# NVlabs/FB-BEV

Measured on NVIDIA B200. Metric: bev_voxels_per_sec, higher is better.
Workload: dtype f32

## Files before the change

### fb-bev_b200/_lib.py

```python
import ctypes
import os
import subprocess

import torch

_HERE = os.path.dirname(os.path.abspath(__file__))
LIB_PATH = os.environ.get("FBBEV_LIB") or os.path.join(
    _HERE, "lib", "libfbbev_b200.so")
CSRC_DIR = os.path.join(_HERE, "csrc")

_p = ctypes.c_void_p
_i32 = ctypes.c_int32
_i64 = ctypes.c_int64
_sz = ctypes.c_size_t

_SIGNATURES = {
    "fbbev_abi_version": (ctypes.c_int, []),
    "fbbev_debug_launch_count": (ctypes.c_longlong, []),
    "fbbev_error_string": (ctypes.c_char_p, [ctypes.c_int]),
    "fbbev_bev_pool_v2_fwd": (ctypes.c_int, [_p] * 7 + [_i32, _i32, _p, _p]),
    "fbbev_bev_pool_v2_dense_workspace_bytes": (
        _sz, [_i32, _i64, _i32, _i32, _i32]),
    "fbbev_bev_pool_v2_fwd_dense": (
        ctypes.c_int,
# ... 49 lines not shown
                              [_p] + [_i32] * 9 + [_p, _p, _sz, _p]),
    "fbbev_history_warp": (ctypes.c_int, [_p, _i64, _p] + [_i32] * 5 +
                           [_p, _i32, _i32, _p]),
    "fbbev_linear_packed_bytes": (ctypes.c_size_t, [_i32, _i32]),
    "fbbev_linear_pack": (ctypes.c_int, [_p, _i32, _i32, _p, _p]),
    "fbbev_linear_fwd_split": (ctypes.c_int, [
        _p, _i64, _p, _i64, _p, _p, _i64, _i32, _i32, _i32, _i32, _p, _i64, _p,
        _i64, _p]),
    "fbbev_linear_fwd": (ctypes.c_int, [
        _p, _i64, _p, _p, _p, _i64, _p, _p, _i64, _i32, _i32, _i32,
        ctypes.c_float, _p, _i64, _p]),
    "fbbev_ffn_supported": (ctypes.c_int, [_i32, _i32]),
    "fbbev_ffn_fwd": (ctypes.c_int, [
        _p, _i64, _p, _p, _p, _p, _p, _i64, _p, _p, _i64, _i32, _i32,
        ctypes.c_float, _p, _i64, _p]),
}
EXPORTED_SYMBOLS = tuple(_SIGNATURES)

ABI_VERSION = 4
_lib = None


class FbbevError(RuntimeError):
    pass


def build(verbose=False):
    cmd = ["make", "-C", CSRC_DIR, "-j", str(min(8, os.cpu_count() or 1))]
    res = subprocess.run(cmd, stdout=subprocess.PIPE, stderr=subprocess.STDOUT,
                         text=True)
# ... 112 lines not shown
```

### fb-bev_b200/csrc/ffn_tf32.cu

```cuda
#include "common.cuh"
#include "tc5.cuh"

namespace fbbev {
namespace ffn {

constexpr int kKB = 40;
constexpr int kChunks = kKB / 4;
constexpr int kTileM = 128;
constexpr int kAPart = kTileM * kKB * 4;
constexpr int kABlock = 2 * kAPart;
constexpr int kAChunkStride = (kTileM / 8) * 128;
constexpr int kThreads = 448;
constexpr int kHC = 80;
constexpr int kMaxE = 80;
constexpr int kMaxHidden = 320;
constexpr int kTmemCols = 512;
constexpr int kSmemLimit = 232448 - 1024;
constexpr int kCtrlBytes = 512 + (kMaxHidden + 3 * kMaxE) * 4;
constexpr int kSlabBytes = kTileM * (kMaxE + 4) * 4;

#ifdef FFN_TRACE
constexpr int kTraceCap = 200;
__device__ long long g_ffn_trace[5 * 2 * kTraceCap];
__device__ int g_ffn_trace_cnt[5];
#define FTRACE_DECL int trn_ = 0;
#define FTRACE_L(lane_, tag)                                                 \
  do {                                                                       \
    if (blockIdx.x == 0 && trn_ < kTraceCap) {                               \
      g_ffn_trace[(lane_) * 2 * kTraceCap + 2 * trn_] = (tag);               \
      g_ffn_trace[(lane_) * 2 * kTraceCap + 2 * trn_ + 1] = clock64();       \
      g_ffn_trace_cnt[lane_] = ++trn_;                                       \
    }                                                                        \
  } while (0)
#else
#define FTRACE_DECL
#define FTRACE_L(lane_, tag) do {} while (0)
#endif

struct Params {
  const float* x;
  const float* w1p;
  const float* b1;
  const float* w2p;
  const float* b2;
  const float* residual;
  const float* gamma;
  const float* beta;
  float* y;
  int M, E, hidden, npad, n_kb1, n_kb2, n_hc, rows_per_cta, wstages;
  int64_t ldx, ldr, ldy;
  float eps;
};

__global__ void __launch_bounds__(kThreads, 1) ffn_tf32_kernel(const Params p) {
  extern __shared__ __align__(1024) unsigned char smem[];
  FTRACE_DECL
  const int warp = threadIdx.x >> 5, lane = threadIdx.x & 31;
  const int npad = p.npad, S = p.wstages;
  const uint32_t w1_stage = 2u * kHC * kKB * 4;
  const uint32_t w2_stage = 2u * (uint32_t)npad * kKB * 4;
  const uint32_t wstage = w1_stage > w2_stage ? w1_stage : w2_stage;
  unsigned char* xa = smem;
  unsigned char* slab_raw = smem + 2 * kABlock;
  unsigned char* wr = slab_raw + kSlabBytes;
  unsigned char* ctrl = wr + (size_t)S * wstage;
  const uint32_t bars = smem_u32(ctrl);
  const uint32_t bar_xfull = bars, bar_xempty = bars + 8;
  const uint32_t bar_yfull = bars + 16, bar_yempty = bars + 24;
  const uint32_t bar_hafull = bars + 32;
  const uint32_t bar_haempty = bars + 48;
  const uint32_t bar_hfull = bars + 64;
  const uint32_t bar_wfull = bars + 128;
  const uint32_t bar_wempty = bars + 160;
  uint32_t* tmem_slot = reinterpret_cast<uint32_t*>(ctrl + 192);
  float* s_b1 = reinterpret_cast<float*>(ctrl + 512);
  float* s_b2 = s_b1 + kMaxHidden;
  float* s_gamma = s_b2 + kMaxE;
  float* s_beta = s_gamma + kMaxE;
  const uint32_t xa_base = smem_u32(xa), wr_base = smem_u32(wr);

  if (warp == 12) {
    if (lane == 0) {
      mbar_init(bar_xfull, 128);
      mbar_init(bar_xempty, 1);
      mbar_init(bar_yfull, 1);
      mbar_init(bar_yempty, 128);
      for (int g = 0; g < 2; ++g) {
        mbar_init(bar_hafull + 8u * g, 128);
        mbar_init(bar_haempty + 8u * g, 1);
      }
      for (int c = 0; c < p.n_hc; ++c) mbar_init(bar_hfull + 8u * c, 1);
      for (int s = 0; s < S; ++s) {
        mbar_init(bar_wfull + 8u * s, 1);
        mbar_init(bar_wempty + 8u * s, 1);
      }
      fence_mbar_init();
    }
    __syncwarp();
    asm volatile(
        "tcgen05.alloc.cta_group::1.sync.aligned.shared::cta.b32 [%0], %1;" ::"r"(
            smem_u32(tmem_slot)),
        "r"(kTmemCols)
        : "memory");
    asm volatile("tcgen05.relinquish_alloc_permit.cta_group::1.sync.aligned;" ::
                     : "memory");
  }
  for (int j = threadIdx.x; j < kMaxHidden; j += kThreads)
    s_b1[j] = (p.b1 && j < p.hidden) ? p.b1[j] : 0.f;
  for (int j = threadIdx.x; j < kMaxE; j += kThreads) {
    s_b2[j] = (p.b2 && j < p.E) ? p.b2[j] : 0.f;
    s_gamma[j] = (p.gamma && j < p.E) ? p.gamma[j] : 1.f;
    s_beta[j] = (p.beta && j < p.E) ? p.beta[j] : 0.f;
  }
  tc_fence_before();
  __syncthreads();
  tc_fence_after();
  const uint32_t tmem_base = *tmem_slot;
  if (threadIdx.x == 0) FTRACE_L(4, 1);
  const int row_begin = blockIdx.x * p.rows_per_cta;
  const int row_end = min(p.M, row_begin + p.rows_per_cta);
  const int n_my = row_end > row_begin ? (row_end - row_begin + kTileM - 1) / kTileM : 0;
  const int stages_per_tile = p.n_hc * p.n_kb1 + p.n_kb2;

  if (warp >= 4 && warp < 8) {
    const int lw = warp - 4;
    const int r_lo = lane & 15, c_lo = lane >> 4;
    auto load_x = [&](int ti) {
      float4 v[2][10];
#pragma unroll
      for (int u = 0; u < 2; ++u) {
        const int g0 = row_begin + ti * kTileM + lw * 32 + r_lo;
        const int col0 = u * kKB + 4 * c_lo;
        const float* b0 = p.x + (size_t)g0 * p.ldx + col0;
        const float* b1 = b0 + (size_t)16 * p.ldx;
        const bool ok0 = u < p.n_kb1 && g0 < row_end;
        const bool ok1 = u < p.n_kb1 && g0 + 16 < row_end;
#pragma unroll
// ... 25 lines not shown
          lo.x = x.x - hi.x; lo.y = x.y - hi.y;
          lo.z = x.z - hi.z; lo.w = x.w - hi.w;
          const uint32_t off =
              (uint32_t)(ch * (kTileM / 8) + (row >> 3)) * 128u + (row & 7) * 16u;
          unsigned char* a = xa + (size_t)u * kABlock + off;
          *reinterpret_cast<float4*>(a) = hi;
          *reinterpret_cast<float4*>(a + kAPart) = lo;
        }
      }
      fence_proxy_async();
      mbar_arrive(bar_xfull);
      if (threadIdx.x == 128) FTRACE_L(0, 120 + ti);
    };
    for (int ti = 0; ti < n_my; ++ti) load_x(ti);
  } else if (warp == 13) {
    const int n_w1 = p.n_hc * p.n_kb1;
    uint32_t it = 0;
    for (int ti = 0; ti < n_my; ++ti) {
      for (int j = 0; j < stages_per_tile; ++j, ++it) {
        const uint32_t s = it % S, ph = (it / S) & 1u;
        const float* src;
        uint32_t bytes;
        if (j < n_w1) {
          src = p.w1p + (size_t)j * (w1_stage / 4u);
          bytes = w1_stage;
        } else {
          src = p.w2p + (size_t)(j - n_w1) * (w2_stage / 4u);
          bytes = w2_stage;
        }
        mbar_wait(bar_wempty + 8u * s, ph ^ 1u);
        if (lane == 0) FTRACE_L(1, 1000 + it);
        if (elect_one()) {
          mbar_arrive_expect_tx(bar_wfull + 8u * s, bytes);
          bulk_g2s(wr_base + s * wstage, src, bytes, bar_wfull + 8u * s);
        }
        __syncwarp();
      }
    }
  } else if (warp == 12) {
    {
      const uint32_t idesc1 = (1u << 4) | (2u << 7) | (2u << 10) |
                              ((uint32_t)(kHC >> 3) << 17) | (8u << 24);
      const uint32_t idesc2 = (1u << 4) | (2u << 7) | (2u << 10) |
                              ((uint32_t)(npad >> 3) << 17) | (8u << 24);
      const uint32_t lbo_b1 = (uint32_t)kHC * 16u, lbo_b2 = (uint32_t)npad * 16u;
      const uint32_t w1_part = (uint32_t)kHC * kKB * 4;
      const uint32_t w2_part = (uint32_t)npad * kKB * 4;
      const uint32_t d_y = tmem_base + (uint32_t)p.hidden;
      const uint32_t d_lo = d_y + (uint32_t)npad;
      uint32_t it = 0, hu = 0;
      for (int ti = 0; ti < n_my; ++ti) {
        if (lane == 0) FTRACE_L(2, 200 + ti);
        mbar_wait(bar_xfull, ti & 1);
        tc_fence_after();
        if (lane == 0) FTRACE_L(2, 210 + ti);
        for (int c = 0; c < p.n_hc; ++c) {
          const uint32_t d = tmem_base + (uint32_t)(c * kHC);
          for (int kb = 0; kb < p.n_kb1; ++kb, ++it) {
            const uint32_t s = it % S, ph = (it / S) & 1u;
            mbar_wait(bar_wfull + 8u * s, ph);
            tc_fence_after();
            if (lane == 0) FTRACE_L(2, 2000 + it);
            const uint32_t a_hi = xa_base + (uint32_t)kb * kABlock;
            const uint32_t a_lo = a_hi + kAPart;
            const uint32_t w_hi = wr_base + s * wstage;
            const uint32_t w_lo = w_hi + w1_part;
            if (elect_one()) {
#pragma unroll
// ... 7 lines not shown
              mma_tf32(d, dal, dbh, idesc1, 1u);
              mma_tf32(d, dah, dbl, idesc1, 1u);
            }
            tc_commit(bar_wempty + 8u * s);
            if (kb == p.n_kb1 - 1) {
              tc_commit(bar_hfull + 8u * c);
              if (c == p.n_hc - 1) tc_commit(bar_xempty);
            }
            }
            __syncwarp();
          }
        }
        mbar_wait(bar_yempty, (ti & 1) ^ 1);
        tc_fence_after();
        for (int kb = 0; kb < p.n_kb2; ++kb, ++it, ++hu) {
          const uint32_t s = it % S, ph = (it / S) & 1u;
          const uint32_t g = (uint32_t)kb & 1u, hph = (hu >> 1) & 1u;
          mbar_wait(bar_wfull + 8u * s, ph);
          if (lane == 0) FTRACE_L(2, 2000 + it);
          mbar_wait(bar_hafull + 8u * g, hph);
          tc_fence_after();
          if (lane == 0) FTRACE_L(2, 3000 + it);
          const uint32_t a_hi = tmem_base + (uint32_t)(kb * kKB);
          const uint32_t a_lo = d_lo + g * (uint32_t)kKB;
          const uint32_t w_hi = wr_base + s * wstage;
          const uint32_t w_lo = w_hi + w2_part;
          if (elect_one()) {
#pragma unroll
          for (int k = 0; k < kChunks / 2; ++k) {
            const uint32_t bo = 2u * k * lbo_b2;
            const uint64_t dbh = smem_desc(w_hi + bo, lbo_b2, 128);
            const uint64_t dbl = smem_desc(w_lo + bo, lbo_b2, 128);
            mma_tf32_ts(d_y, a_hi + 8u * k, dbh, idesc2, (kb | k) != 0);
            mma_tf32_ts(d_y, a_lo + 8u * k, dbh, idesc2, 1u);
            mma_tf32_ts(d_y, a_hi + 8u * k, dbl, idesc2, 1u);
          }
          tc_commit(bar_wempty + 8u * s);
          tc_commit(bar_haempty + 8u * g);
          if (kb == p.n_kb2 - 1) tc_commit(bar_yfull);
          }
          __syncwarp();
        }
        if (lane == 0) FTRACE_L(2, 220 + ti);
      }
    }
    __syncwarp();
  } else if (warp != 13) {
    const uint32_t grp = warp >> 3;
    const int q = warp & 3;
    const int gt = q * 32 + lane;
    const uint32_t lane_base = tmem_base + ((uint32_t)(q * 32) << 16);
    const int E = p.E;
    if (grp == 1) {
      const uint32_t t_lo = lane_base + (uint32_t)(p.hidden + npad);
      uint32_t use = 0;
      for (int ti = 0; ti < n_my; ++ti) {
        for (int kb = 0; kb < p.n_kb2; ++kb, ++use) {
// ... 24 lines not shown
          tmem_st16(tl, lo);
          tmem_st16(tl + 16u, lo + 16);
          tmem_st8(tl + 32u, lo + 32);
          tmem_st_wait();
          tc_fence_before();
          mbar_arrive(bar_hafull + 8u * g);
          if (threadIdx.x == 256) FTRACE_L(3, 6000 + use);
        }
      }
    } else {
      const int pitch = E + 4;
      float* slab = reinterpret_cast<float*>(slab_raw);
      float* my_row = slab + (size_t)gt * pitch;
      const uint32_t ty = lane_base + (uint32_t)p.hidden;
      const int nc16 = npad >> 4;
      for (int ti = 0; ti < n_my; ++ti) {
        const int row0 = row_begin + ti * kTileM;
        const bool in_range = row0 + gt < row_end;
        bulk_wait_read0();
        asm volatile("bar.sync 1, 128;" ::: "memory");
        if (p.residual) {
          const int crow = gt >> 2, cq = gt & 3;
#pragma unroll 1
          for (int c = 0; c < nc16; ++c) {
            const int col = 16 * c + 4 * cq;
#pragma unroll
            for (int i = 0; i < 4; ++i) {
              const int r = crow + 32 * i;
              const bool ok = row0 + r < row_end && col < E;
              const float* src = p.residual +
                                 (size_t)(ok ? row0 + r : row_begin) * p.ldr +
                                 (ok ? col : 0);
              const uint32_t dst = smem_u32(slab + (size_t)r * pitch + col);
              asm volatile("cp.async.cg.shared.global [%0], [%1], 16, %2;" ::"r"(dst),
                           "l"(src), "r"(ok ? 16 : 0)
                           : "memory");
            }
          }
          asm volatile("cp.async.commit_group;" ::: "memory");
        }
        if (threadIdx.x == 0) FTRACE_L(4, 300 + ti);
        mbar_wait(bar_yfull, ti & 1);
        tc_fence_after();
        if (threadIdx.x == 0) FTRACE_L(4, 310 + ti);
        if (p.residual) {
          asm volatile("cp.async.wait_group 0;" ::: "memory");
          asm volatile("bar.sync 1, 128;" ::: "memory");
        }
        float sum = 0.f, sq = 0.f, shiftK = 0.f;
#pragma unroll 1
        for (int c = 0; c < nc16; ++c) {
          float v[16];
          tmem_ld16(ty + 16u * c, v);
          tmem_ld_wait();
          if (c == nc16 - 1) {
            tc_fence_before();
            mbar_arrive(bar_yempty);
          }
#pragma unroll
          for (int j = 0; j < 4; ++j) {
            const int col = 16 * c + 4 * j;
            if (col < E) {
              const float4 bb = *reinterpret_cast<const float4*>(s_b2 + col);
              float4 t = make_float4(v[4 * j] + bb.x, v[4 * j + 1] + bb.y,
                                     v[4 * j + 2] + bb.z, v[4 * j + 3] + bb.w);
              float4* cell = reinterpret_cast<float4*>(my_row + col);
              if (p.residual) {
                const float4 r = *cell;
                t.x += r.x; t.y += r.y; t.z += r.z; t.w += r.w;
              }
              *cell = t;
              if (col == 0) shiftK = t.x;
              const float a = t.x - shiftK, b = t.y - shiftK, cc = t.z - shiftK,
                          d = t.w - shiftK;
              sum += (a + b) + (cc + d);
              sq += (a * a + b * b) + (cc * cc + d * d);
            }
          }
        }
        if (p.gamma) {
          const float dm = sum / (float)E;
          const float mean = shiftK + dm;
          const float var = fmaxf(sq / (float)E - dm * dm, 0.f);
          const float rstd = rsqrtf(var + p.eps);
          const float4* g4 = reinterpret_cast<const float4*>(s_gamma);
          const float4* b4 = reinterpret_cast<const float4*>(s_beta);
#pragma unroll 4
          for (int j = 0; j < (E >> 2); ++j) {
            float4* cell = reinterpret_cast<float4*>(my_row + 4 * j);
            const float4 t = *cell, g = g4[j], b = b4[j];
            *cell = make_float4(fmaf((t.x - mean) * rstd, g.x, b.x),
                                fmaf((t.y - mean) * rstd, g.y, b.y),
                                fmaf((t.z - mean) * rstd, g.z, b.z),
                                fmaf((t.w - mean) * rstd, g.w, b.w));
          }
        }
        if (in_range) {
          fence_proxy_async();
          bulk_s2g(p.y + (size_t)(row0 + gt) * p.ldy, smem_u32(my_row),
                   (uint32_t)E * 4u);
        }
        bulk_commit();
        if (threadIdx.x == 0) FTRACE_L(4, 320 + ti);
      }
      bulk_wait0();
      if (threadIdx.x == 0) FTRACE_L(4, 330);
    }
  }

  tc_fence_before();
  __syncthreads();
// ... 19 lines not shown
  cudaMemcpyFromSymbol(out, ffn::g_ffn_trace,
                       sizeof(long long) * 5 * 2 * ffn::kTraceCap);
  return ffn::kTraceCap;
}
#endif

FBBEV_API int fbbev_ffn_supported(int32_t embed, int32_t hidden) {
  return embed > 0 && embed <= ffn::kMaxE && embed % 4 == 0 && hidden > 0 &&
                 hidden % ffn::kHC == 0 &&
                 hidden + ffn::pad16(embed) + 2 * ffn::kKB <= ffn::kTmemCols &&
                 hidden <= ffn::kMaxHidden
             ? 1
             : 0;
}

FBBEV_API int fbbev_ffn_fwd(const float* x, int64_t ldx, const float* w1_packed,
                            const float* b1, const float* w2_packed,
                            const float* b2, const float* residual, int64_t ldr,
                            const float* ln_weight, const float* ln_bias,
                            int64_t m, int32_t embed, int32_t hidden,
                            float ln_eps, float* y, int64_t ldy,
                            fbbev_stream_t stream) {
  if (!x || !w1_packed || !w2_packed || !y || m < 0)
    return FBBEV_ERR_INVALID_ARGUMENT;
  if ((ln_weight == nullptr) != (ln_bias == nullptr))
    return FBBEV_ERR_INVALID_ARGUMENT;
  if (!fbbev_ffn_supported(embed, hidden) || m > (int64_t)1 << 30)
    return FBBEV_ERR_UNSUPPORTED;
  if (ldx < embed || ldy < embed || (residual && ldr < embed) || ldx % 4 ||
      ldy % 4 || (residual && ldr % 4))
    return FBBEV_ERR_INVALID_ARGUMENT;
  if ((reinterpret_cast<uintptr_t>(x) | reinterpret_cast<uintptr_t>(y) |
       reinterpret_cast<uintptr_t>(w1_packed) |
       reinterpret_cast<uintptr_t>(w2_packed) |
       reinterpret_cast<uintptr_t>(residual)) & 15)
    return FBBEV_ERR_INVALID_ARGUMENT;
  if (m == 0) return FBBEV_OK;
  ffn::Params p;
  p.x = x; p.w1p = w1_packed; p.b1 = b1; p.w2p = w2_packed; p.b2 = b2;
  p.residual = residual; p.gamma = ln_weight; p.beta = ln_bias; p.y = y;
  p.M = (int)m; p.E = embed; p.hidden = hidden; p.npad = ffn::pad16(embed);
  p.n_kb1 = (embed + ffn::kKB - 1) / ffn::kKB;
  p.n_kb2 = hidden / ffn::kKB;
  p.n_hc = hidden / ffn::kHC;
  p.ldx = ldx; p.ldr = ldr; p.ldy = ldy; p.eps = ln_eps;
  const size_t w1_stage = 2 * (size_t)ffn::kHC * ffn::kKB * 4;
  const size_t w2_stage = 2 * (size_t)p.npad * ffn::kKB * 4;
  const size_t wstage = w1_stage > w2_stage ? w1_stage : w2_stage;
  const size_t fixed =
      2 * (size_t)ffn::kABlock + ffn::kSlabBytes + ffn::kCtrlBytes;
  int S = (int)((ffn::kSmemLimit - fixed) / wstage);
  S = S > 4 ? 4 : S;
  if (S < 2) return FBBEV_ERR_UNSUPPORTED;
  p.wstages = S;
  const size_t smem = fixed + (size_t)S * wstage;
  static int n_sm = 0;
  if (n_sm == 0) {
    int dev = 0;
    cudaGetDevice(&dev);
    cudaDeviceGetAttribute(&n_sm, cudaDevAttrMultiProcessorCount, dev);
    if (n_sm <= 0) n_sm = 148;
  }
  const int n_tiles = (int)ceil_div64(m, ffn::kTileM);
  const int tiles_per_cta = (int)ceil_div64(n_tiles, n_sm);
  p.rows_per_cta = tiles_per_cta * ffn::kTileM;
  const int grid = (int)ceil_div64(m, p.rows_per_cta);
  static size_t allowed = 0;
  if (smem > allowed) {
    cudaError_t e = cudaFuncSetAttribute(
        ffn::ffn_tf32_kernel, cudaFuncAttributeMaxDynamicSharedMemorySize,
        (int)smem);
    if (e != cudaSuccess) return (int)e;
    allowed = smem;
  }
  count_launch();
  ffn::ffn_tf32_kernel<<<grid, ffn::kThreads, smem, as_stream(stream)>>>(p);
  return launch_status();
}
```

### fb-bev_b200/csrc/linear_tf32.cu

```cuda
#include "common.cuh"
#include "tc5.cuh"

namespace fbbev {

constexpr int kKB = 40;
constexpr int kChunks = kKB / 4;
constexpr int kTileM = 128;
constexpr int kAPart = kTileM * kKB * 4;
constexpr int kAChunkStride = (kTileM / 8) * 128;
constexpr int kLinThreads = 448;
constexpr int kMaxN = 192;
constexpr int kTmemCols = 512;
constexpr int kSmemLimit = 232448 - 1024;
constexpr int kSlabPitch = 20;
constexpr int kSlabBytes = 2 * kTileM * kSlabPitch * 4;
constexpr int kCtrlBytes = 256 + 3 * kMaxN * 4;

#ifdef LIN_TRACE
__device__ long long g_trace[512];
__device__ int g_trace_n;
#define TRACE_DECL __shared__ long long s_trace[8][64]; __shared__ int s_trace_n[8];
#define TRACE(lane_, tag)                                                    \
  do {                                                                       \
    if (blockIdx.x == 0) {                                                   \
// ... 256 lines not shown
    for (int ti = 0; ti < n_my; ++ti, ++tc) {
      if ((tc & 1u) != grp) continue;
      const uint32_t aph = (tc >> 1) & 1u;
      const int row0 = row_begin + ti * kTileM;
      const uint32_t taddr =
          tmem_base + ((uint32_t)(q * 32) << 16) + grp * (uint32_t)npad;
      if (LN) {
        bulk_wait_read0();
        group_sync();
        if (p.residual) {
#pragma unroll 1
          for (int c = 0; c < nc16; ++c) {
            const int col = 16 * c + 4 * cq;
#pragma unroll
            for (int i = 0; i < 4; ++i) {
              const int r = crow + 32 * i;
              const bool ok = row0 + r < row_end && col < N;
              const float* src = p.residual +
                                 (size_t)(ok ? row0 + r : row_begin) * p.ldr +
                                 (ok ? col : 0);
              const uint32_t dst = smem_u32(slab + (size_t)r * pitch + col);
              asm volatile("cp.async.cg.shared.global [%0], [%1], 16, %2;" ::"r"(dst),
                           "l"(src), "r"(ok ? 16 : 0)
                           : "memory");
            }
          }
          asm volatile("cp.async.commit_group;" ::: "memory");
        }
        if (gt == 0) TRACE(3 + grp, 600 + tc);
        mbar_wait(bar_tfull + 8u * grp, aph);
        tc_fence_after();
        if (gt == 0) TRACE(3 + grp, 700 + tc);
// ... 286 lines not shown
```

### fb-bev_b200/ops/linear.py

```python
import torch

from .. import _lib

MAX_N = 192


def _pack(weight):
    key = (weight.data_ptr(), weight._version, tuple(weight.shape), weight.device)
    hit = getattr(weight, "_fbbev_packed", None)
    if hit is not None and hit[0] == key:
        return hit[1]
    L = _lib.lib()
    n, k = weight.shape
    w = weight.detach().contiguous().float()
    blocks = []
    for n0 in range(0, n, MAX_N):
        n1 = min(n, n0 + MAX_N)
        nbytes = L.fbbev_linear_packed_bytes(n1 - n0, k)
        buf = torch.empty(nbytes // 4, dtype=torch.float32, device=w.device)
        _lib.check(L.fbbev_linear_pack(_lib.ptr(w[n0:n1]), n1 - n0, k, _lib.ptr(buf),
                                       _lib.stream_ptr(w.device)), "fbbev_linear_pack")
        blocks.append((n0, n1, buf))
    try:
        weight._fbbev_packed = (key, blocks)
# ... 149 lines not shown
    w1p = _pack_ffn_w1(w1)
    (_, _, w2p), = _pack(w2)
    _lib.check(_lib.lib().fbbev_ffn_fwd(
        _lib.ptr(x2), x2.stride(0), _lib.ptr(w1p),
        _lib.ptr(b1.detach().contiguous()) if b1 is not None else None,
        _lib.ptr(w2p),
        _lib.ptr(b2.detach().contiguous()) if b2 is not None else None,
        _lib.ptr(r2), r2.stride(0) if r2 is not None else 0,
        _lib.ptr(ln_weight) if ln_weight is not None else None,
        _lib.ptr(ln_bias) if ln_bias is not None else None,
        m, embed, hidden, float(eps), _lib.ptr(y), y.stride(0),
        _lib.stream_ptr(x.device)), "fbbev_ffn_fwd")
    return y.view(*lead, embed)


class LinearTF32Function(torch.autograd.Function):

    @staticmethod
    def forward(ctx, x, weight, bias, relu, residual):
        assert not (relu and residual is not None)
        y = linear_fused(
            x.detach(), weight.detach(),
            None if bias is None else bias.detach(), relu=relu,
            residual=None if residual is None else residual.detach())
        ctx.relu = relu
        ctx.has_bias = bias is not None
        ctx.has_res = residual is not None
        ctx.save_for_backward(x, weight, y if relu else None)
        return y

# ... 23 lines not shown
```

### fb-bev_b200/view_transformation/backward_projection.py

```python
import copy
import math
import os
import warnings

import torch
import torch.nn as nn
import torch.nn.functional as F

from ..ops import linear as _linear_ops
from .forward_projection import inv3x3_many
from ..ops import ms_deform_attn as _msda_ops
from ..ops.ms_deform_attn import (MultiScaleDeformableAttnFunction_fp32,
                                  bev_mask_fold,
                                  da_spatial_cross_attention_core,
                                  da_spatial_cross_attention_core_autograd,
                                  ms_deform_attn_fused, ms_deform_attn_unfused,
                                  needs_grad)
from ..registry import (BaseModule, build_attention,
                        build_feedforward_network, build_positional_encoding,
                        build_transformer, build_transformer_layer,
                        build_transformer_layer_sequence, register)

__all__ = ['BackwardProjection', 'BEVFormer', 'bevformer_encoder',
           'BEVFormerEncoderLayer', 'MyCustomBaseTransformerLayer',
# ... 427 lines not shown
        if self.layer_scale is None and _fused_linear_on(slots, self.dropout):
            return _linear(self.output_proj, slots, residual=inp_residual,
                           norm=post_norm)
        slots = self.output_proj(slots)
        if self.layer_scale is None:
            out = self.dropout(slots) + inp_residual
        else:
            out = self.dropout(self.layer_scale * slots) + inp_residual
        return out if post_norm is None else post_norm(out)

    def forward(self, query, key, value, residual=None, query_pos=None,
                key_padding_mask=None, reference_points=None,
                spatial_shapes=None, reference_points_cam=None,
                level_start_index=None, flag='encoder', bev_query_depth=None,
                pred_img_depth=None, bev_mask=None, per_cam_mask_list=None,
                post_norm=None, **kwargs):
        query = query.float()
        if key is None:
            key = query
        if value is None:
            value = key
        inp_residual = query if residual is None else residual
        side_event = kwargs.get('side_event')
        if side_event is not None and query.is_cuda:
            torch.cuda.current_stream(query.device).wait_event(side_event)
        sca_prepared = (kwargs.get('sca_prepared') or {}).get(id(self))
        if bev_mask is not None:
            if self.rebatch_bev_mask or not query.is_cuda:
                if query_pos is not None:
                    query = query + query_pos.float()
                return self._forward_rebatch(
                    query, value, inp_residual, key_padding_mask,
                    spatial_shapes, reference_points_cam, level_start_index,
                    bev_query_depth, pred_img_depth, bev_mask,
                    per_cam_mask_list, post_norm)
            per_cam_mask_list = bev_mask_fold(per_cam_mask_list, bev_mask)
            sca_prepared = None

        da = self.deformable_attention
        B, N, DC, H, W = pred_img_depth.shape
        depth_prob = pred_img_depth.reshape(B * N, DC, H * W).permute(0, 2, 1)
        v = (kwargs.get('projected_values') or {}).get(id(self))
        if v is None:
# ... 1 lines not shown
        offsets, logits = da.project_query(
            query, None if query_pos is None else query_pos.float())
        if bev_query_depth.dim() == 5:
            bev_query_depth = bev_query_depth[..., 0]
        if needs_grad(v, depth_prob, offsets, logits):
            slots = da_spatial_cross_attention_core_autograd(
                v, depth_prob, reference_points_cam, bev_query_depth,
                per_cam_mask_list, offsets, logits, spatial_shapes,
                level_start_index, self.dbound, da.num_Z_anchors)
        else:
            slots = da_spatial_cross_attention_core(
                v, depth_prob, reference_points_cam, bev_query_depth,
                per_cam_mask_list, offsets, logits, spatial_shapes,
                level_start_index, self.dbound, da.num_Z_anchors,
                prepared=sca_prepared)
        return self._finish(slots, inp_residual, post_norm)

    def project_camera_value(self, value):
        num_cams, n_value, bs, E = value.shape
        value = value.permute(2, 0, 1, 3).reshape(bs * num_cams, n_value, E)
        return self.deformable_attention.project_value(value.float())

    def _forward_rebatch(self, query, value, inp_residual, key_padding_mask,
                         spatial_shapes, reference_points_cam,
                         level_start_index, bev_query_depth, pred_img_depth,
                         bev_mask, per_cam_mask_list, post_norm=None):
        N, B, nq, Z, _ = bev_query_depth.shape
        _, _, DC, H, W = pred_img_depth.shape
        depth_q = bev_query_depth.permute(1, 0, 2, 3, 4)
        depth_prob = pred_img_depth.reshape(B * N, DC, H * W).permute(0, 2, 1)
# ... 160 lines not shown
                    attn_mask=attn_masks[attn_index],
                    key_padding_mask=bev_mask, reference_points=ref_2d,
                    spatial_shapes=_const_tensor(((bev_h, bev_w),),
                                                 query.device),
                    level_start_index=_const_tensor((0,), query.device),
                    post_norm=fold, bev_w=bev_w, **kwargs)
                attn_index += 1
                identity = query
                skip_norm = fold is not None
            elif op == 'norm':
                if not skip_norm:
                    query = self.norms[norm_index](query)
                skip_norm = False
                norm_index += 1
            elif op == 'cross_attn':
                query = self.attentions[attn_index](
                    query, key, value, identity if self.pre_norm else None,
                    query_pos=bev_pos, key_pos=key_pos,
                    reference_points=ref_3d,
                    reference_points_cam=reference_points_cam,
                    attn_mask=attn_masks[attn_index],
                    key_padding_mask=key_padding_mask,
                    spatial_shapes=spatial_shapes,
                    level_start_index=level_start_index,
                    bev_query_depth=bev_query_depth,
                    pred_img_depth=pred_img_depth, bev_mask=bev_mask,
                    per_cam_mask_list=per_cam_mask_list, post_norm=fold,
                    **kwargs)
                attn_index += 1
                identity = query
                skip_norm = fold is not None
            elif op == 'ffn':
                query = self.ffns[ffn_index](
                    query, identity if self.pre_norm else None,
                    post_norm=fold)
                ffn_index += 1
                skip_norm = fold is not None
        return query


@register('TRANSFORMER_LAYER_SEQUENCE')
class bevformer_encoder(BaseModule):

    fused_geometry = os.environ.get('FBBEV_EXACT_GEOMETRY', '0') != '1'
    side_stream = os.environ.get('FBBEV_SIDE_STREAM', '1') == '1'

    @staticmethod
    def _side(device):
        key = str(device)
        if key not in _SIDE_STREAMS:
            _SIDE_STREAMS[key] = torch.cuda.Stream(device=device)
        return _SIDE_STREAMS[key]

# ... 302 lines not shown
```

### include/fbbev_b200.h

```cpp
#ifndef FBBEV_B200_H_
#define FBBEV_B200_H_

#include <stddef.h>
#include <stdint.h>

#ifdef __cplusplus
extern "C" {
#endif

#define FBBEV_OK 0
#define FBBEV_ERR_INVALID_ARGUMENT (-1)
#define FBBEV_ERR_WORKSPACE_TOO_SMALL (-2)
#define FBBEV_ERR_UNSUPPORTED (-3)

#define FBBEV_ABI_VERSION 4

typedef void* fbbev_stream_t;

int fbbev_abi_version(void);
long long fbbev_debug_launch_count(void);
const char* fbbev_error_string(int code);


int fbbev_bev_pool_v2_fwd(const float* depth, const float* feat,
// ... 189 lines not shown
int fbbev_linear_fwd_split(const float* x, int64_t ldx, const float* x_add,
                           int64_t ldx_add, const float* packed,
                           const float* bias, int64_t m, int32_t k, int32_t n,
                           int32_t n_split, int32_t relu, float* y0,
                           int64_t ldy0, float* y1, int64_t ldy1,
                           fbbev_stream_t stream);

int fbbev_ffn_supported(int32_t embed, int32_t hidden);
int fbbev_ffn_fwd(const float* x, int64_t ldx, const float* w1_packed,
                  const float* b1, const float* w2_packed, const float* b2,
                  const float* residual, int64_t ldr, const float* ln_weight,
                  const float* ln_bias, int64_t m, int32_t embed,
                  int32_t hidden, float ln_eps, float* y, int64_t ldy,
                  fbbev_stream_t stream);


int fbbev_history_warp(const float* history, int64_t history_batch_stride,
                       const float* flow, int32_t n, int32_t mc, int32_t Z,
                       int32_t H, int32_t W, float* out, int32_t c_total,
                       int32_t ch_offset, fbbev_stream_t stream);

#ifdef __cplusplus
}
#endif
#endif
```

Before: 1.549 billion.

## Fuse cross-attention output projection and LayerNorm into the FFN tcgen05 kernel

Adds a prologue GEMM stage to the TF32 FFN kernel that computes the cross-attention output projection, adds the bias and residual, and applies the first LayerNorm. The normalized rows are written back as the FFN input and residual, and the next tile's prologue is interleaved with the current tile's second GEMM. The encoder layer routes cross_attn, norm, ffn and norm through this single kernel when the configuration matches. This removes a separate linear launch and the global round trip of the intermediate activation. In exchange it adds extra pipeline barriers, shared-memory control space, and ordering complexity between the bulk stores and the residual reloads.

```diff
diff --git a/fb-bev_b200/_lib.py b/fb-bev_b200/_lib.py
--- a/fb-bev_b200/_lib.py
+++ b/fb-bev_b200/_lib.py
@@ -87,6 +87,9 @@
     "fbbev_ffn_fwd": (ctypes.c_int, [
         _p, _i64, _p, _p, _p, _p, _p, _i64, _p, _p, _i64, _i32, _i32,
         ctypes.c_float, _p, _i64, _p]),
+    "fbbev_proj_ln_ffn_fwd": (ctypes.c_int, [
+        _p, _i64, _p, _p, _p, _i64, _p, _p, ctypes.c_float, _p, _p, _p, _p,
+        _p, _p, _i64, _i32, _i32, ctypes.c_float, _p, _i64, _p]),
 }
 EXPORTED_SYMBOLS = tuple(_SIGNATURES)
 
diff --git a/fb-bev_b200/csrc/ffn_tf32.cu b/fb-bev_b200/csrc/ffn_tf32.cu
--- a/fb-bev_b200/csrc/ffn_tf32.cu
+++ b/fb-bev_b200/csrc/ffn_tf32.cu
@@ -16,7 +16,7 @@
 constexpr int kMaxHidden = 320;
 constexpr int kTmemCols = 512;
 constexpr int kSmemLimit = 232448 - 1024;
-constexpr int kCtrlBytes = 512 + (kMaxHidden + 3 * kMaxE) * 4;
+constexpr int kCtrlBytes = 512 + (kMaxHidden + 6 * kMaxE) * 4;
 constexpr int kSlabBytes = kTileM * (kMaxE + 4) * 4;
 
 #ifdef FFN_TRACE
@@ -47,9 +47,14 @@
   const float* gamma;
   const float* beta;
   float* y;
+  const float* wop;
+  const float* bo;
+  const float* residual0;
+  const float* gamma0;
+  const float* beta0;
   int M, E, hidden, npad, n_kb1, n_kb2, n_hc, rows_per_cta, wstages;
-  int64_t ldx, ldr, ldy;
-  float eps;
+  int64_t ldx, ldr, ldy, ldr0;
+  float eps, eps0;
 };
 
 __global__ void __launch_bounds__(kThreads, 1) ffn_tf32_kernel(const Params p) {
@@ -70,6 +75,8 @@
   const uint32_t bar_hafull = bars + 32;
   const uint32_t bar_haempty = bars + 48;
   const uint32_t bar_hfull = bars + 64;
+  const uint32_t bar_pfull = bars + 112;
+  const uint32_t bar_qfull = bars + 120;
   const uint32_t bar_wfull = bars + 128;
   const uint32_t bar_wempty = bars + 160;
   uint32_t* tmem_slot = reinterpret_cast<uint32_t*>(ctrl + 192);
@@ -77,6 +84,10 @@
   float* s_b2 = s_b1 + kMaxHidden;
   float* s_gamma = s_b2 + kMaxE;
   float* s_beta = s_gamma + kMaxE;
+  float* s_bo = s_beta + kMaxE;
+  float* s_gamma0 = s_bo + kMaxE;
+  float* s_beta0 = s_gamma0 + kMaxE;
+  const bool pro = p.wop != nullptr;
   const uint32_t xa_base = smem_u32(xa), wr_base = smem_u32(wr);
 
   if (warp == 12) {
@@ -90,6 +101,8 @@
         mbar_init(bar_haempty + 8u * g, 1);
       }
       for (int c = 0; c < p.n_hc; ++c) mbar_init(bar_hfull + 8u * c, 1);
+      mbar_init(bar_pfull, 1);
+      mbar_init(bar_qfull, 128);
       for (int s = 0; s < S; ++s) {
         mbar_init(bar_wfull + 8u * s, 1);
         mbar_init(bar_wempty + 8u * s, 1);
@@ -111,6 +124,9 @@
     s_b2[j] = (p.b2 && j < p.E) ? p.b2[j] : 0.f;
     s_gamma[j] = (p.gamma && j < p.E) ? p.gamma[j] : 1.f;
     s_beta[j] = (p.beta && j < p.E) ? p.beta[j] : 0.f;
+    s_bo[j] = (p.bo && j < p.E) ? p.bo[j] : 0.f;
+    s_gamma0[j] = (p.gamma0 && j < p.E) ? p.gamma0[j] : 1.f;
+    s_beta0[j] = (p.beta0 && j < p.E) ? p.beta0[j] : 0.f;
   }
   tc_fence_before();
   __syncthreads();
@@ -120,7 +136,8 @@
   const int row_begin = blockIdx.x * p.rows_per_cta;
   const int row_end = min(p.M, row_begin + p.rows_per_cta);
   const int n_my = row_end > row_begin ? (row_end - row_begin + kTileM - 1) / kTileM : 0;
-  const int stages_per_tile = p.n_hc * p.n_kb1 + p.n_kb2;
+  const int n_w0 = pro ? p.n_kb1 : 0;
+  const int stages_per_tile = n_w0 + p.n_hc * p.n_kb1 + p.n_kb2;
 
   if (warp >= 4 && warp < 8) {
     const int lw = warp - 4;
@@ -176,27 +193,30 @@
     };
     for (int ti = 0; ti < n_my; ++ti) load_x(ti);
   } else if (warp == 13) {
-    const int n_w1 = p.n_hc * p.n_kb1;
     uint32_t it = 0;
+    auto issue = [&](const float* src, uint32_t bytes) {
+      const uint32_t s = it % S, ph = (it / S) & 1u;
+      mbar_wait(bar_wempty + 8u * s, ph ^ 1u);
+      if (lane == 0) FTRACE_L(1, 1000 + it);
+      if (elect_one()) {
+        mbar_arrive_expect_tx(bar_wfull + 8u * s, bytes);
+        bulk_g2s(wr_base + s * wstage, src, bytes, bar_wfull + 8u * s);
+      }
+      __syncwarp();
+      ++it;
+    };
+    auto issue_wo = [&]() {
+      for (int kb = 0; kb < p.n_kb1; ++kb)
+        issue(p.wop + (size_t)kb * (w2_stage / 4u), w2_stage);
+    };
+    if (pro && n_my > 0) issue_wo();
     for (int ti = 0; ti < n_my; ++ti) {
-      for (int j = 0; j < stages_per_tile; ++j, ++it) {
-        const uint32_t s = it % S, ph = (it / S) & 1u;
-        const float* src;
-        uint32_t bytes;
-        if (j < n_w1) {
-          src = p.w1p + (size_t)j * (w1_stage / 4u);
-          bytes = w1_stage;
-        } else {
-          src = p.w2p + (size_t)(j - n_w1) * (w2_stage / 4u);
-          bytes = w2_stage;
-        }
-        mbar_wait(bar_wempty + 8u * s, ph ^ 1u);
-        if (lane == 0) FTRACE_L(1, 1000 + it);
-        if (elect_one()) {
-          mbar_arrive_expect_tx(bar_wfull + 8u * s, bytes);
-          bulk_g2s(wr_base + s * wstage, src, bytes, bar_wfull + 8u * s);
-        }
-        __syncwarp();
+      for (int j = 0; j < p.n_hc * p.n_kb1; ++j)
+        issue(p.w1p + (size_t)j * (w1_stage / 4u), w1_stage);
+      for (int kb = 0; kb <= p.n_kb2; ++kb) {
+        if (kb == 2 && pro && ti + 1 < n_my) issue_wo();
+        if (kb == p.n_kb2) break;
+        issue(p.w2p + (size_t)kb * (w2_stage / 4u), w2_stage);
       }
     }
   } else if (warp == 12) {
@@ -211,9 +231,39 @@
       const uint32_t d_y = tmem_base + (uint32_t)p.hidden;
       const uint32_t d_lo = d_y + (uint32_t)npad;
       uint32_t it = 0, hu = 0;
+      auto gemm0 = [&](int t) {
+        mbar_wait(bar_xfull, t & 1);
+        tc_fence_after();
+        for (int kb = 0; kb < p.n_kb1; ++kb, ++it) {
+          const uint32_t s = it % S, ph = (it / S) & 1u;
+          mbar_wait(bar_wfull + 8u * s, ph);
+          tc_fence_after();
+          const uint32_t a_hi = xa_base + (uint32_t)kb * kABlock;
+          const uint32_t a_lo = a_hi + kAPart;
+          const uint32_t w_hi = wr_base + s * wstage;
+          const uint32_t w_lo = w_hi + w2_part;
+          if (elect_one()) {
+#pragma unroll
+          for (int k = 0; k < kChunks / 2; ++k) {
+            const uint32_t ao = 2u * k * kAChunkStride, bo = 2u * k * lbo_b2;
+            const uint64_t dah = smem_desc(a_hi + ao, kAChunkStride, 128);
+            const uint64_t dal = smem_desc(a_lo + ao, kAChunkStride, 128);
+            const uint64_t dbh = smem_desc(w_hi + bo, lbo_b2, 128);
+            const uint64_t dbl = smem_desc(w_lo + bo, lbo_b2, 128);
+            mma_tf32(tmem_base, dah, dbh, idesc2, (kb | k) != 0);
+            mma_tf32(tmem_base, dal, dbh, idesc2, 1u);
+            mma_tf32(tmem_base, dah, dbl, idesc2, 1u);
+          }
+          tc_commit(bar_wempty + 8u * s);
+          if (kb == p.n_kb1 - 1) tc_commit(bar_pfull);
+          }
+          __syncwarp();
+        }
+      };
+      if (pro && n_my > 0) gemm0(0);
       for (int ti = 0; ti < n_my; ++ti) {
         if (lane == 0) FTRACE_L(2, 200 + ti);
-        mbar_wait(bar_xfull, ti & 1);
+        mbar_wait(pro ? bar_qfull : bar_xfull, ti & 1);
         tc_fence_after();
         if (lane == 0) FTRACE_L(2, 210 + ti);
         for (int c = 0; c < p.n_hc; ++c) {
@@ -251,6 +301,7 @@
         mbar_wait(bar_yempty, (ti & 1) ^ 1);
         tc_fence_after();
         for (int kb = 0; kb < p.n_kb2; ++kb, ++it, ++hu) {
+          if (kb == 2 && pro && ti + 1 < n_my) gemm0(ti + 1);
           const uint32_t s = it % S, ph = (it / S) & 1u;
           const uint32_t g = (uint32_t)kb & 1u, hph = (hu >> 1) & 1u;
           mbar_wait(bar_wfull + 8u * s, ph);
@@ -278,6 +329,7 @@
           }
           __syncwarp();
         }
+        if (p.n_kb2 == 2 && pro && ti + 1 < n_my) gemm0(ti + 1);
         if (lane == 0) FTRACE_L(2, 220 + ti);
       }
     }
@@ -332,58 +384,49 @@
       float* my_row = slab + (size_t)gt * pitch;
       const uint32_t ty = lane_base + (uint32_t)p.hidden;
       const int nc16 = npad >> 4;
-      for (int ti = 0; ti < n_my; ++ti) {
-        const int row0 = row_begin + ti * kTileM;
-        const bool in_range = row0 + gt < row_end;
-        bulk_wait_read0();
-        asm volatile("bar.sync 1, 128;" ::: "memory");
-        if (p.residual) {
-          const int crow = gt >> 2, cq = gt & 3;
+      auto prefetch_rows = [&](const float* src0, int64_t ld, int row0) {
+        const int crow = gt >> 2, cq = gt & 3;
 #pragma unroll 1
-          for (int c = 0; c < nc16; ++c) {
-            const int col = 16 * c + 4 * cq;
-#pragma unroll
-            for (int i = 0; i < 4; ++i) {
-              const int r = crow + 32 * i;
-              const bool ok = row0 + r < row_end && col < E;
-              const float* src = p.residual +
-                                 (size_t)(ok ? row0 + r : row_begin) * p.ldr +
-                                 (ok ? col : 0);
-              const uint32_t dst = smem_u32(slab + (size_t)r * pitch + col);
-              asm volatile("cp.async.cg.shared.global [%0], [%1], 16, %2;" ::"r"(dst),
-                           "l"(src), "r"(ok ? 16 : 0)
-                           : "memory");
-            }
-          }
-          asm volatile("cp.async.commit_group;" ::: "memory");
-        }
-        if (threadIdx.x == 0) FTRACE_L(4, 300 + ti);
-        mbar_wait(bar_yfull, ti & 1);
-        tc_fence_after();
-        if (threadIdx.x == 0) FTRACE_L(4, 310 + ti);
-        if (p.residual) {
-          asm volatile("cp.async.wait_group 0;" ::: "memory");
-          asm volatile("bar.sync 1, 128;" ::: "memory");
-        }
+        for (int c = 0; c < nc16; ++c) {
+          const int col = 16 * c + 4 * cq;
+#pragma unroll
+          for (int i = 0; i < 4; ++i) {
+            if (col >= E) break;
+            const int r = crow + 32 * i;
+            const bool ok = row0 + r < row_end;
+            const float* src = src0 +
+                               (size_t)(ok ? row0 + r : row_begin) * ld +
+                               (ok ? col : 0);
+            const uint32_t dst = smem_u32(slab + (size_t)r * pitch + col);
+            asm volatile("cp.async.cg.shared.global [%0], [%1], 16, %2;" ::"r"(dst),
+                         "l"(src), "r"(ok ? 16 : 0)
+                         : "memory");
+          }
+        }
+        asm volatile("cp.async.commit_group;" ::: "memory");
+      };
+      auto row_ln = [&](uint32_t tcol, const float* bias, bool add_res,
+                        const float* gamma, const float* beta, float eps,
+                        uint32_t release) {
         float sum = 0.f, sq = 0.f, shiftK = 0.f;
 #pragma unroll 1
         for (int c = 0; c < nc16; ++c) {
           float v[16];
-          tmem_ld16(ty + 16u * c, v);
+          tmem_ld16(tcol + 16u * c, v);
           tmem_ld_wait();
-          if (c == nc16 - 1) {
+          if (c == nc16 - 1 && release) {
             tc_fence_before();
-            mbar_arrive(bar_yempty);
+            mbar_arrive(release);
           }
 #pragma unroll
           for (int j = 0; j < 4; ++j) {
             const int col = 16 * c + 4 * j;
             if (col < E) {
-              const float4 bb = *reinterpret_cast<const float4*>(s_b2 + col);
+              const float4 bb = *reinterpret_cast<const float4*>(bias + col);
               float4 t = make_float4(v[4 * j] + bb.x, v[4 * j + 1] + bb.y,
                                      v[4 * j + 2] + bb.z, v[4 * j + 3] + bb.w);
               float4* cell = reinterpret_cast<float4*>(my_row + col);
-              if (p.residual) {
+              if (add_res) {
                 const float4 r = *cell;
                 t.x += r.x; t.y += r.y; t.z += r.z; t.w += r.w;
               }
@@ -396,13 +439,13 @@
             }
           }
         }
-        if (p.gamma) {
+        if (gamma) {
           const float dm = sum / (float)E;
           const float mean = shiftK + dm;
           const float var = fmaxf(sq / (float)E - dm * dm, 0.f);
-          const float rstd = rsqrtf(var + p.eps);
-          const float4* g4 = reinterpret_cast<const float4*>(s_gamma);
-          const float4* b4 = reinterpret_cast<const float4*>(s_beta);
+          const float rstd = rsqrtf(var + eps);
+          const float4* g4 = reinterpret_cast<const float4*>(gamma);
+          const float4* b4 = reinterpret_cast<const float4*>(beta);
 #pragma unroll 4
           for (int j = 0; j < (E >> 2); ++j) {
             float4* cell = reinterpret_cast<float4*>(my_row + 4 * j);
@@ -413,6 +456,76 @@
                                 fmaf((t.w - mean) * rstd, g.w, b.w));
           }
         }
+      };
+      auto prologue = [&](int t) {
+        const int row0 = row_begin + t * kTileM;
+        bulk_wait_read0();
+        asm volatile("bar.sync 1, 128;" ::: "memory");
+        if (p.residual0) prefetch_rows(p.residual0, p.ldr0, row0);
+        mbar_wait(bar_pfull, t & 1);
+        tc_fence_after();
+        if (p.residual0) {
+          asm volatile("cp.async.wait_group 0;" ::: "memory");
+          asm volatile("bar.sync 1, 128;" ::: "memory");
+        }
+        row_ln(lane_base, s_bo, p.residual0 != nullptr,
+               p.gamma0 ? s_gamma0 : nullptr, s_beta0, p.eps0, 0u);
+#pragma unroll
+        for (int u = 0; u < 2; ++u) {
+          if (u >= p.n_kb1) break;
+#pragma unroll
+          for (int ch = 0; ch < kChunks; ++ch) {
+            const int col = u * kKB + 4 * ch;
+            if (col < E) {
+              const float4 x = *reinterpret_cast<const float4*>(my_row + col);
+              float4 hi, lo;
+              hi.x = __uint_as_float(__float_as_uint(x.x) & 0xFFFFE000u);
+              hi.y = __uint_as_float(__float_as_uint(x.y) & 0xFFFFE000u);
+              hi.z = __uint_as_float(__float_as_uint(x.z) & 0xFFFFE000u);
+              hi.w = __uint_as_float(__float_as_uint(x.w) & 0xFFFFE000u);
+              lo.x = x.x - hi.x; lo.y = x.y - hi.y;
+              lo.z = x.z - hi.z; lo.w = x.w - hi.w;
+              const uint32_t off =
+                  (uint32_t)(ch * (kTileM / 8) + (gt >> 3)) * 128u + (gt & 7) * 16u;
+              unsigned char* a = xa + (size_t)u * kABlock + off;
+              *reinterpret_cast<float4*>(a) = hi;
+              *reinterpret_cast<float4*>(a + kAPart) = lo;
+            }
+          }
+        }
+        fence_proxy_async();
+        tc_fence_before();
+        mbar_arrive(bar_qfull);
+        if (row0 + gt < row_end)
+          bulk_s2g(p.y + (size_t)(row0 + gt) * p.ldy, smem_u32(my_row),
+                   (uint32_t)E * 4u);
+        bulk_commit();
+      };
+      const float* res = pro ? p.y : p.residual;
+      const int64_t ldres = pro ? p.ldy : p.ldr;
+      if (pro && n_my > 0) prologue(0);
+      for (int ti = 0; ti < n_my; ++ti) {
+        const int row0 = row_begin + ti * kTileM;
+        const bool in_range = row0 + gt < row_end;
+        if (pro && ti + 1 < n_my) prologue(ti + 1);
+        if (pro) {
+          bulk_wait0();
+          asm volatile("fence.proxy.async.global;" ::: "memory");
+        } else {
+          bulk_wait_read0();
+        }
+        asm volatile("bar.sync 1, 128;" ::: "memory");
+        if (res) prefetch_rows(res, ldres, row0);
+        if (threadIdx.x == 0) FTRACE_L(4, 300 + ti);
+        mbar_wait(bar_yfull, ti & 1);
+        tc_fence_after();
+        if (threadIdx.x == 0) FTRACE_L(4, 310 + ti);
+        if (res) {
+          asm volatile("cp.async.wait_group 0;" ::: "memory");
+          asm volatile("bar.sync 1, 128;" ::: "memory");
+        }
+        row_ln(ty, s_b2, res != nullptr, p.gamma ? s_gamma : nullptr, s_beta,
+               p.eps, bar_yempty);
         if (in_range) {
           fence_proxy_async();
           bulk_s2g(p.y + (size_t)(row0 + gt) * p.ldy, smem_u32(my_row),
@@ -462,36 +575,7 @@
              : 0;
 }
 
-FBBEV_API int fbbev_ffn_fwd(const float* x, int64_t ldx, const float* w1_packed,
-                            const float* b1, const float* w2_packed,
-                            const float* b2, const float* residual, int64_t ldr,
-                            const float* ln_weight, const float* ln_bias,
-                            int64_t m, int32_t embed, int32_t hidden,
-                            float ln_eps, float* y, int64_t ldy,
-                            fbbev_stream_t stream) {
-  if (!x || !w1_packed || !w2_packed || !y || m < 0)
-    return FBBEV_ERR_INVALID_ARGUMENT;
-  if ((ln_weight == nullptr) != (ln_bias == nullptr))
-    return FBBEV_ERR_INVALID_ARGUMENT;
-  if (!fbbev_ffn_supported(embed, hidden) || m > (int64_t)1 << 30)
-    return FBBEV_ERR_UNSUPPORTED;
-  if (ldx < embed || ldy < embed || (residual && ldr < embed) || ldx % 4 ||
-      ldy % 4 || (residual && ldr % 4))
-    return FBBEV_ERR_INVALID_ARGUMENT;
-  if ((reinterpret_cast<uintptr_t>(x) | reinterpret_cast<uintptr_t>(y) |
-       reinterpret_cast<uintptr_t>(w1_packed) |
-       reinterpret_cast<uintptr_t>(w2_packed) |
-       reinterpret_cast<uintptr_t>(residual)) & 15)
-    return FBBEV_ERR_INVALID_ARGUMENT;
-  if (m == 0) return FBBEV_OK;
-  ffn::Params p;
-  p.x = x; p.w1p = w1_packed; p.b1 = b1; p.w2p = w2_packed; p.b2 = b2;
-  p.residual = residual; p.gamma = ln_weight; p.beta = ln_bias; p.y = y;
-  p.M = (int)m; p.E = embed; p.hidden = hidden; p.npad = ffn::pad16(embed);
-  p.n_kb1 = (embed + ffn::kKB - 1) / ffn::kKB;
-  p.n_kb2 = hidden / ffn::kKB;
-  p.n_hc = hidden / ffn::kHC;
-  p.ldx = ldx; p.ldr = ldr; p.ldy = ldy; p.eps = ln_eps;
+static int ffn_launch(ffn::Params& p, cudaStream_t st) {
   const size_t w1_stage = 2 * (size_t)ffn::kHC * ffn::kKB * 4;
   const size_t w2_stage = 2 * (size_t)p.npad * ffn::kKB * 4;
   const size_t wstage = w1_stage > w2_stage ? w1_stage : w2_stage;
@@ -509,10 +593,10 @@
     cudaDeviceGetAttribute(&n_sm, cudaDevAttrMultiProcessorCount, dev);
     if (n_sm <= 0) n_sm = 148;
   }
-  const int n_tiles = (int)ceil_div64(m, ffn::kTileM);
+  const int n_tiles = (int)ceil_div64(p.M, ffn::kTileM);
   const int tiles_per_cta = (int)ceil_div64(n_tiles, n_sm);
   p.rows_per_cta = tiles_per_cta * ffn::kTileM;
-  const int grid = (int)ceil_div64(m, p.rows_per_cta);
+  const int grid = (int)ceil_div64(p.M, p.rows_per_cta);
   static size_t allowed = 0;
   if (smem > allowed) {
     cudaError_t e = cudaFuncSetAttribute(
@@ -522,6 +606,85 @@
     allowed = smem;
   }
   count_launch();
-  ffn::ffn_tf32_kernel<<<grid, ffn::kThreads, smem, as_stream(stream)>>>(p);
+  ffn::ffn_tf32_kernel<<<grid, ffn::kThreads, smem, st>>>(p);
   return launch_status();
 }
+
+static int ffn_check(const float* x, int64_t ldx, const float* w1_packed,
+                     const float* w2_packed, const float* residual,
+                     int64_t ldr, const float* ln_weight, const float* ln_bias,
+                     int64_t m, int32_t embed, int32_t hidden, const float* y,
+                     int64_t ldy) {
+  if (!x || !w1_packed || !w2_packed || !y || m < 0)
+    return FBBEV_ERR_INVALID_ARGUMENT;
+  if ((ln_weight == nullptr) != (ln_bias == nullptr))
+    return FBBEV_ERR_INVALID_ARGUMENT;
+  if (!fbbev_ffn_supported(embed, hidden) || m > (int64_t)1 << 30)
+    return FBBEV_ERR_UNSUPPORTED;
+  if (ldx < embed || ldy < embed || (residual && ldr < embed) || ldx % 4 ||
+      ldy % 4 || (residual && ldr % 4))
+    return FBBEV_ERR_INVALID_ARGUMENT;
+  if ((reinterpret_cast<uintptr_t>(x) | reinterpret_cast<uintptr_t>(y) |
+       reinterpret_cast<uintptr_t>(w1_packed) |
+       reinterpret_cast<uintptr_t>(w2_packed) |
+       reinterpret_cast<uintptr_t>(residual)) & 15)
+    return FBBEV_ERR_INVALID_ARGUMENT;
+  return FBBEV_OK;
+}
+
+static void ffn_params(ffn::Params& p, const float* x, int64_t ldx,
+                       const float* w1_packed, const float* b1,
+                       const float* w2_packed, const float* b2,
+                       const float* ln_weight, const float* ln_bias, int64_t m,
+                       int32_t embed, int32_t hidden, float ln_eps, float* y,
+                       int64_t ldy) {
+  p = ffn::Params{};
+  p.x = x; p.w1p = w1_packed; p.b1 = b1; p.w2p = w2_packed; p.b2 = b2;
+  p.gamma = ln_weight; p.beta = ln_bias; p.y = y;
+  p.M = (int)m; p.E = embed; p.hidden = hidden; p.npad = ffn::pad16(embed);
+  p.n_kb1 = (embed + ffn::kKB - 1) / ffn::kKB;
+  p.n_kb2 = hidden / ffn::kKB;
+  p.n_hc = hidden / ffn::kHC;
+  p.ldx = ldx; p.ldy = ldy; p.eps = ln_eps;
+}
+
+FBBEV_API int fbbev_ffn_fwd(const float* x, int64_t ldx, const float* w1_packed,
+                            const float* b1, const float* w2_packed,
+                            const float* b2, const float* residual, int64_t ldr,
+                            const float* ln_weight, const float* ln_bias,
+                            int64_t m, int32_t embed, int32_t hidden,
+                            float ln_eps, float* y, int64_t ldy,
+                            fbbev_stream_t stream) {
+  const int rc = ffn_check(x, ldx, w1_packed, w2_packed, residual, ldr,
+                           ln_weight, ln_bias, m, embed, hidden, y, ldy);
+  if (rc != FBBEV_OK) return rc;
+  if (m == 0) return FBBEV_OK;
+  ffn::Params p;
+  ffn_params(p, x, ldx, w1_packed, b1, w2_packed, b2, ln_weight, ln_bias, m,
+             embed, hidden, ln_eps, y, ldy);
+  p.residual = residual; p.ldr = ldr;
+  return ffn_launch(p, as_stream(stream));
+}
+
+FBBEV_API int fbbev_proj_ln_ffn_fwd(
+    const float* s, int64_t lds, const float* wo_packed, const float* bo,
+    const float* residual0, int64_t ldr0, const float* ln0_weight,
+    const float* ln0_bias, float ln0_eps, const float* w1_packed,
+    const float* b1, const float* w2_packed, const float* b2,
+    const float* ln_weight, const float* ln_bias, int64_t m, int32_t embed,
+    int32_t hidden, float ln_eps, float* y, int64_t ldy,
+    fbbev_stream_t stream) {
+  const int rc = ffn_check(s, lds, w1_packed, w2_packed, residual0, ldr0,
+                           ln_weight, ln_bias, m, embed, hidden, y, ldy);
+  if (rc != FBBEV_OK) return rc;
+  if (!wo_packed || (ln0_weight == nullptr) != (ln0_bias == nullptr) ||
+      (reinterpret_cast<uintptr_t>(wo_packed) & 15))
+    return FBBEV_ERR_INVALID_ARGUMENT;
+  if (m == 0) return FBBEV_OK;
+  ffn::Params p;
+  ffn_params(p, s, lds, w1_packed, b1, w2_packed, b2, ln_weight, ln_bias, m,
+             embed, hidden, ln_eps, y, ldy);
+  p.wop = wo_packed; p.bo = bo; p.residual0 = residual0; p.ldr0 = ldr0;
+  p.gamma0 = ln0_weight; p.beta0 = ln0_bias; p.eps0 = ln0_eps;
+  return ffn_launch(p, as_stream(stream));
+}
diff --git a/fb-bev_b200/csrc/linear_tf32.cu b/fb-bev_b200/csrc/linear_tf32.cu
--- a/fb-bev_b200/csrc/linear_tf32.cu
+++ b/fb-bev_b200/csrc/linear_tf32.cu
@@ -294,8 +294,9 @@
             const int col = 16 * c + 4 * cq;
 #pragma unroll
             for (int i = 0; i < 4; ++i) {
+              if (col >= N) break;
               const int r = crow + 32 * i;
-              const bool ok = row0 + r < row_end && col < N;
+              const bool ok = row0 + r < row_end;
               const float* src = p.residual +
                                  (size_t)(ok ? row0 + r : row_begin) * p.ldr +
                                  (ok ? col : 0);
diff --git a/fb-bev_b200/ops/linear.py b/fb-bev_b200/ops/linear.py
--- a/fb-bev_b200/ops/linear.py
+++ b/fb-bev_b200/ops/linear.py
@@ -187,6 +187,36 @@
     return y.view(*lead, embed)
 
 
+def proj_ln_ffn(s, wo, bo, residual0, ln0, w1, b1, w2, b2, ln=None):
+    _lib.require_cuda(s)
+    hidden, embed = w1.shape
+    assert s.shape[-1] == embed and tuple(wo.shape) == (embed, embed)
+    assert tuple(w2.shape) == (embed, hidden)
+    lead = s.shape[:-1]
+    s2 = _rows(s, embed)
+    m = s2.shape[0]
+    r2 = _rows(residual0, embed) if residual0 is not None else None
+    y = torch.empty((m, embed), dtype=torch.float32, device=s.device)
+    (_, _, wop), = _pack(wo)
+    w1p = _pack_ffn_w1(w1)
+    (_, _, w2p), = _pack(w2)
+
+    def vec(t):
+        return _lib.ptr(t.detach().contiguous()) if t is not None else None
+
+    _lib.check(_lib.lib().fbbev_proj_ln_ffn_fwd(
+        _lib.ptr(s2), s2.stride(0), _lib.ptr(wop), vec(bo),
+        _lib.ptr(r2), r2.stride(0) if r2 is not None else 0,
+        vec(ln0.weight), vec(ln0.bias), float(ln0.eps),
+        _lib.ptr(w1p), vec(b1), _lib.ptr(w2p), vec(b2),
+        vec(None if ln is None else ln.weight),
+        vec(None if ln is None else ln.bias),
+        m, embed, hidden, 1e-5 if ln is None else float(ln.eps),
+        _lib.ptr(y), y.stride(0), _lib.stream_ptr(s.device)),
+        "fbbev_proj_ln_ffn_fwd")
+    return y.view(*lead, embed)
+
+
 class LinearTF32Function(torch.autograd.Function):
 
     @staticmethod
diff --git a/fb-bev_b200/view_transformation/backward_projection.py b/fb-bev_b200/view_transformation/backward_projection.py
--- a/fb-bev_b200/view_transformation/backward_projection.py
+++ b/fb-bev_b200/view_transformation/backward_projection.py
@@ -465,7 +465,7 @@
                 spatial_shapes=None, reference_points_cam=None,
                 level_start_index=None, flag='encoder', bev_query_depth=None,
                 pred_img_depth=None, bev_mask=None, per_cam_mask_list=None,
-                post_norm=None, **kwargs):
+                post_norm=None, return_slots=False, **kwargs):
         query = query.float()
         if key is None:
             key = query
@@ -478,6 +478,7 @@
         sca_prepared = (kwargs.get('sca_prepared') or {}).get(id(self))
         if bev_mask is not None:
             if self.rebatch_bev_mask or not query.is_cuda:
+                assert not return_slots
                 if query_pos is not None:
                     query = query + query_pos.float()
                 return self._forward_rebatch(
@@ -509,6 +510,8 @@
                 per_cam_mask_list, offsets, logits, spatial_shapes,
                 level_start_index, self.dbound, da.num_Z_anchors,
                 prepared=sca_prepared)
+        if return_slots:
+            return slots
         return self._finish(slots, inp_residual, post_norm)
 
     def project_camera_value(self, value):
@@ -699,7 +702,8 @@
                 skip_norm = False
                 norm_index += 1
             elif op == 'cross_attn':
-                query = self.attentions[attn_index](
+                chain = self._chain_fused(query, attn_index, bev_mask)
+                out = self.attentions[attn_index](
                     query, key, value, identity if self.pre_norm else None,
                     query_pos=bev_pos, key_pos=key_pos,
                     reference_points=ref_3d,
@@ -711,7 +715,15 @@
                     bev_query_depth=bev_query_depth,
                     pred_img_depth=pred_img_depth, bev_mask=bev_mask,
                     per_cam_mask_list=per_cam_mask_list, post_norm=fold,
-                    **kwargs)
+                    **(dict(return_slots=True) if chain else {}), **kwargs)
+                if chain:
+                    attn, ffn = self.attentions[attn_index], self.ffns[0]
+                    fc1, fc2 = ffn.layers[0][0], ffn.layers[-2]
+                    return _linear_ops.proj_ln_ffn(
+                        out, attn.output_proj.weight, attn.output_proj.bias,
+                        query, self.norms[norm_index], fc1.weight, fc1.bias,
+                        fc2.weight, fc2.bias, self.norms[norm_index + 1])
+                query = out
                 attn_index += 1
                 identity = query
                 skip_norm = fold is not None
@@ -722,6 +734,36 @@
                 ffn_index += 1
                 skip_norm = fold is not None
         return query
+
+    def _chain_fused(self, query, attn_index, bev_mask):
+        if (os.environ.get('FBBEV_CHAIN_FUSED', '1') != '1' or
+                os.environ.get('FBBEV_FFN_FUSED', '1') != '1' or
+                tuple(self.operation_order) != ('self_attn', 'norm',
+                                                'cross_attn', 'norm',
+                                                'ffn', 'norm') or
+                torch.is_grad_enabled()):
+            return False
+        attn, ffn = self.attentions[attn_index], self.ffns[0]
+        if not (isinstance(attn, DA_SpatialCrossAttention) and
+                attn.layer_scale is None and
+                not (bev_mask is not None and attn.rebatch_bev_mask)):
+            return False
+        if not (isinstance(ffn, FFN) and ffn.num_fcs == 2 and
+                ffn.add_identity and
+                isinstance(ffn.layers[0][1], nn.ReLU)):
+            return False
+        drops = [m for m in ffn.layers.modules() if isinstance(m, nn.Dropout)]
+        if not _fused_linear_on(query, attn.dropout, ffn.dropout_layer, *drops):
+            return False
+        E = query.shape[-1]
+        for norm in self.norms[1:3]:
+            if not (isinstance(norm, nn.LayerNorm) and
+                    tuple(norm.normalized_shape) == (E,) and
+                    norm.weight is not None and norm.bias is not None):
+                return False
+        fc1, fc2 = ffn.layers[0][0], ffn.layers[-2]
+        return (tuple(attn.output_proj.weight.shape) == (E, E) and
+                _linear_ops.ffn_supported(query, fc1.weight, fc2.weight))
 
 
 @register('TRANSFORMER_LAYER_SEQUENCE')
diff --git a/include/fbbev_b200.h b/include/fbbev_b200.h
--- a/include/fbbev_b200.h
+++ b/include/fbbev_b200.h
@@ -227,6 +227,17 @@
                   int32_t hidden, float ln_eps, float* y, int64_t ldy,
                   fbbev_stream_t stream);
 
+int fbbev_proj_ln_ffn_fwd(const float* s, int64_t lds, const float* wo_packed,
+                          const float* bo, const float* residual0,
+                          int64_t ldr0, const float* ln0_weight,
+                          const float* ln0_bias, float ln0_eps,
+                          const float* w1_packed, const float* b1,
+                          const float* w2_packed, const float* b2,
+                          const float* ln_weight, const float* ln_bias,
+                          int64_t m, int32_t embed, int32_t hidden,
+                          float ln_eps, float* y, int64_t ldy,
+                          fbbev_stream_t stream);
+
 
 int fbbev_history_warp(const float* history, int64_t history_batch_stride,
                        const float* flow, int32_t n, int32_t mc, int32_t Z,
```

Result: faster. 1.576 billion, median of 6 (+1.7%).
